# blackle/Megalania

Hardware: AMD Instinct MI355X
Metric: SA neighbour-cost evals/s (higher is better)
Workload: dtype u64

## Files before the change

megalania_amd/csrc/mgl_api.hip:

```cpp
#include "mgl_kernels.hip"
#include "mgl_kernels2.hip"
#include "mgl_kernels3.hip"
#include "mgl_kernels4.hip"
#include "mgl_kernels5.hip"
#include "mgl_pbuild.hip"
#include "mgl_index.hip"
#include "mgl_matchfinder.hip"
#include "mgl_optimal.hip"
#include "mgl_adaptive.hip"
#include "mgl_props.hip"
#include "../../include/megalania_hip.h"

#include <math.h>
#include <stdio.h>
#include <stdlib.h>
#include <string.h>
#include <string>
#include <vector>

static const uint16_t k_cost_table[2048] = {
#include "mgl_cost_table.inc"
};

#define MGL_MAX_INPUT 176000000ull
// ... 412 lines not shown
			hipStream_t st = (h & 1u) ? sa->stream2 : sa->stream;
			hipLaunchKernelGGL((k_neighbours2<false, MGL_NBR_PICK>), dim3((j1 - j0 + sa->pick_waves - 1) / sa->pick_waves), dim3(64 * sa->pick_waves),
			                   (MGL_PICK_T_GLOBAL ? 0u : 4096u) + sa->pick_waves * sa->per_wave_pick, st, sa->ctx,
			                   sa->b2, sa->base.ctl, sa->cfg.seed, step_override, K, sa->nbr, sa->per_wave_pick, sa->d_todo, sa->d_counts,
			                   (unsigned long long*)nullptr, sa->big, sa->d_pickrec, j0, j1, sa->d_pickstate); NBR_TRACE("k_neighbours2<false, MGL_NBR_PICK>");
			hipLaunchKernelGGL((k_neighbours2<false, MGL_NBR_REST>), dim3(j1 - j0), dim3(64), sa->per_wave_rest, st, sa->ctx,
			                   sa->b2, sa->base.ctl, sa->cfg.seed, step_override, K, sa->nbr, sa->per_wave_rest, sa->d_todo, sa->d_counts,
			                   g_prof_big ? (unsigned long long*)nullptr : sa->d_prof, sa->big, sa->d_pickrec, j0, j1, sa->d_pickstate); NBR_TRACE("k_neighbours2<false, MGL_NBR_REST>");
			HIPCHK(hipEventRecord(sa->ev_rest[h], st));
		}
		HIPCHK(hipGetLastError());
		for (uint32_t h = 0; h < slices; h++) {
			const uint32_t j0 = (uint32_t)((uint64_t)K * h / slices), j1 = (uint32_t)((uint64_t)K * (h + 1) / slices);
			HIPCHK(hipStreamWaitEvent(sa->stream3, sa->ev_rest[h], 0));
			if (sa->time_sim_step >= 0 && h < 2) HIPCHK(hipEventRecord(sim_event(sa, 4 * (size_t)sa->time_sim_step + 2 * h), sa->stream3));
			if (sa->count_traffic)
				hipLaunchKernelGGL(k_sim<true>, dim3(j1 - j0), dim3(64 * sa->sim_waves), sim_lds_regular, sa->stream3, sa->ctx, sa->b2, sa->base.ctl,
				                   sa->nbr, sa->big, j0, j1, sa->d_todo3, sa->d_counts + 4, sa->d_traffic);
			else
				hipLaunchKernelGGL(k_sim<false>, dim3(j1 - j0), dim3(64 * sa->sim_waves), sim_lds_regular, sa->stream3, sa->ctx, sa->b2, sa->base.ctl,
				                   sa->nbr, sa->big, j0, j1, sa->d_todo3, sa->d_counts + 4, (unsigned long long*)nullptr);
			NBR_TRACE("k_sim");
			if (sa->time_sim_step >= 0 && h < 2) HIPCHK(hipEventRecord(sim_event(sa, 4 * (size_t)sa->time_sim_step + 2 * h + 1), sa->stream3));
		}
		HIPCHK(hipEventRecord(sa->ev_sim, sa->stream3));
		for (uint32_t h = 1; h < slices; h += 2) HIPCHK(hipStreamWaitEvent(sa->stream, sa->ev_rest[h], 0));
	}
	if (!sa->split_nbr || sa->form_single) {
		hipLaunchKernelGGL((k_neighbours2<false, MGL_NBR_FULL>), dim3(blocks2), dim3(64 * sa->waves_per_block2), sa->nbr2_lds, sa->stream, sa->ctx,
		                   sa->b2, sa->base.ctl, sa->cfg.seed, step_override, K, sa->nbr, sa->per_wave2, sa->d_todo, sa->d_counts,
		                   sa->d_prof, sa->big, sa->d_pickrec, 0u, K, sa->d_pickstate); NBR_TRACE("k_neighbours2<false, MGL_NBR_FULL>");
	}
	const uint32_t bigblocks = sa->big.slots < 1024u ? sa->big.slots : 1024u;
	const uint32_t big_lds = 4096u + sa->per_wave2 + 12u * MGL_BIG_CAP + MGL_COOP_BYTES;
	hipLaunchKernelGGL((k_neighbours2<true, MGL_NBR_FULL>), dim3(bigblocks), dim3(64 * sa->big_waves), big_lds, sa->stream, sa->ctx,
	                   sa->b2, sa->base.ctl, sa->cfg.seed, step_override, K, sa->nbr, sa->per_wave2, sa->d_todo2, sa->d_counts + 1,
	                   g_prof_big ? sa->d_prof : (unsigned long long*)nullptr, sa->big, split_now ? sa->d_pickrec : (uint4*)nullptr, 0u, K, sa->d_pickstate); NBR_TRACE("k_neighbours2<true, MGL_NBR_FULL>");
	if (split_now) {
		HIPCHK(hipStreamWaitEvent(sa->stream, sa->ev_sim, 0));
		BigScratch late = sa->big;
		late.todo_in = sa->d_todo3; late.todo_in_count = sa->d_counts + 4;
		late.cont = nullptr;
		hipLaunchKernelGGL((k_neighbours2<true, MGL_NBR_FULL>), dim3(bigblocks < 64u ? bigblocks : 64u), dim3(64 * sa->big_waves), big_lds, sa->stream, sa->ctx,
		                   sa->b2, sa->base.ctl, sa->cfg.seed, step_override, K, sa->nbr, sa->per_wave2, sa->d_todo2, sa->d_counts + 1,
		                   (unsigned long long*)nullptr, late, sa->d_pickrec, 0u, K, sa->d_pickstate); NBR_TRACE("k_neighbours2<true, MGL_NBR_FULL>");
	}
	const uint32_t blocks = (K + sa->waves_per_block - 1) / sa->waves_per_block;
	hipLaunchKernelGGL(k_neighbours, dim3(blocks < 256u ? blocks : 256u), dim3(64 * sa->waves_per_block), sa->nbr_lds, sa->stream, sa->ctx, sa->base.v,
	                   (const Control*)sa->base.ctl, sa->cfg.seed, step_override, K, sa->nbr, sa->per_wave_bytes,
	                   (const uint32_t*)sa->d_todo2, (const uint32_t*)(sa->d_counts + 1)); NBR_TRACE("k_neighbours");
	HIPCHK(hipGetLastError());
	return MGL_OK;
}

static int import_slab(mgl_sa* sa, const mgl_packet* packets, mgl_pk* d_slab)
{
	HIPCHK(hipMemcpyAsync(sa->d_aos, packets, sizeof(mgl_packet) * (size_t)sa->n, hipMemcpyHostToDevice, sa->stream));
	hipLaunchKernelGGL(k_import, dim3(1024), dim3(256), 0, sa->stream, (const uint32_t*)sa->d_aos, d_slab, sa->n);
	HIPCHK(hipGetLastError());
	return MGL_OK;
}
static int export_slab(mgl_sa* sa, const mgl_pk* d_slab, mgl_packet* packets)
{
	hipLaunchKernelGGL(k_export, dim3(1024), dim3(256), 0, sa->stream, d_slab, sa->d_aos, sa->n);
	HIPCHK(hipGetLastError());
	HIPCHK(hipMemcpyAsync(packets, sa->d_aos, sizeof(mgl_packet) * (size_t)sa->n, hipMemcpyDeviceToHost, sa->stream));
	HIPCHK(hipStreamSynchronize(sa->stream));
// ... 363 lines not shown
			sa->per_wave_rest = (fixed + lists + 15u) & ~15u;
		}
		{
			BigScratch& g = sa->big;
			memset(&g, 0, sizeof g);
			g.chg_cap = sa->chg_cap;
			g.cap = MGL_BIG_CAP; g.uctx_cap = ckpt_elems; g.slots = (uint32_t)(K > 512 ? K : 512);
			HIPCHK(hipMalloc(&g.ins_key, sizeof(uint16_t) * (size_t)g.cap * g.slots));
			HIPCHK(hipMalloc(&g.rem_key, sizeof(uint16_t) * (size_t)g.cap * g.slots));
			HIPCHK(hipMalloc(&g.ins_pos, sizeof(uint32_t) * (size_t)g.cap * g.slots));
			HIPCHK(hipMalloc(&g.rem_pos, sizeof(uint32_t) * (size_t)g.cap * g.slots));
			HIPCHK(hipMalloc(&g.uctx, sizeof(uint16_t) * (size_t)g.uctx_cap * g.slots));
			HIPCHK(hipMalloc(&sa->d_todo2, sizeof(uint32_t) * (K + 1)));
			HIPCHK(hipMemset(sa->d_todo2, 0, sizeof(uint32_t) * (K + 1)));
		}
		{
			uint32_t best_w = 1, best_total = 0;
			for (uint32_t w = 1; w <= 8; w++) {
				const uint32_t bytes = 4096u + w * sa->per_wave2;
				if (bytes > 160u * 1024u) break;
				const uint32_t tot = (160u * 1024u / bytes) * w;
				if (tot > best_total) { best_total = tot; best_w = w; }
			}
			(void)best_w;
			sa->waves_per_block2 = 1;
		}
		sa->nbr2_lds = 4096u + sa->waves_per_block2 * sa->per_wave2;
		sa->build_lds = 4096u + ckpt_elems * 2u + ckpt_elems * 8u;
		HIPCHK(hipMalloc(&sa->d_counts, sizeof(uint32_t) * 16));
		HIPCHK(hipMemset(sa->d_counts, 0, sizeof(uint32_t) * 16));
		HIPCHK(hipMalloc(&sa->d_todo3, sizeof(uint32_t) * (K + 1)));
		HIPCHK(hipMemset(sa->d_todo3, 0, sizeof(uint32_t) * (K + 1)));
		sa->big.todo_in = sa->d_todo; sa->big.todo_in_count = sa->d_counts; sa->big.spill_ctr = sa->d_counts + 2;
		HIPCHK(hipFuncSetAttribute((const void*)k_neighbours2<false, MGL_NBR_FULL>, hipFuncAttributeMaxDynamicSharedMemorySize, (int)sa->nbr2_lds));
		HIPCHK(hipFuncSetAttribute((const void*)k_neighbours2<false, MGL_NBR_PICK>, hipFuncAttributeMaxDynamicSharedMemorySize, 160 * 1024));
		HIPCHK(hipFuncSetAttribute((const void*)k_neighbours2<false, MGL_NBR_REST>, hipFuncAttributeMaxDynamicSharedMemorySize, (int)sa->nbr2_lds));
		HIPCHK(hipFuncSetAttribute((const void*)k_neighbours2<true, MGL_NBR_FULL>, hipFuncAttributeMaxDynamicSharedMemorySize, (int)(4096u + sa->per_wave2 + 12u * MGL_BIG_CAP + MGL_COOP_BYTES)));
		HIPCHK(hipMalloc(&sa->d_pickrec, sizeof(uint4) * K));
		HIPCHK(hipMalloc(&sa->d_pickstate, sizeof(uint4) * 2 * K));
		sa->split_nbr = getenv("MGL_NO_SPLIT") == nullptr;
		if (sa->split_nbr) {
			BigScratch& g = sa->big;
			HIPCHK(hipMalloc(&g.sim_hdr, sizeof(uint4) * (size_t)K));
			HIPCHK(hipMalloc(&g.sim_keys, sizeof(uint16_t) * 2u * sa->chg_cap * (size_t)K));
			HIPCHK(hipMalloc(&g.sim_pos, sizeof(uint32_t) * 2u * sa->chg_cap * (size_t)K));
			HIPCHK(hipMemset(g.sim_hdr, 0xFF, sizeof(uint4) * (size_t)K));
			if (getenv("MGL_NO_CONT") == nullptr) {
				HIPCHK(hipMalloc(&g.cont, sizeof(uint32_t) * MGL_CONT_WORDS * (size_t)g.slots));
				HIPCHK(hipMemset(g.cont, 0, sizeof(uint32_t) * MGL_CONT_WORDS * (size_t)g.slots));
			}
		}
		if (getenv("MGL_SIMW")) { const int w = atoi(getenv("MGL_SIMW")); if (w == 1 || w == 2 || w == 4 || w == 8) sa->sim_waves = (uint32_t)w; }
		sa->adaptive = sa->split_nbr && getenv("MGL_NO_ADAPT") == nullptr;
		sa->form_single = !sa->split_nbr;
		sa->pick_waves = getenv("MGL_PICK_WAVES") ? (uint32_t)atoi(getenv("MGL_PICK_WAVES")) : 0u;
		if (sa->pick_waves != 1 && sa->pick_waves != 2 && sa->pick_waves != 4 && sa->pick_waves != 8) sa->pick_waves = 0;
		{
			uint32_t best_w = 1, best_resident = 0;
			for (uint32_t w = 1; w <= 8; w *= 2) {
				const uint32_t bytes = (MGL_PICK_T_GLOBAL ? 0u : 4096u) + w * sa->per_wave_pick;
				if (bytes > 160u * 1024u) break;
				const uint32_t resident = (160u * 1024u / ((bytes + 1279u) / 1280u * 1280u)) * w;
				if (resident > best_resident) { best_resident = resident; best_w = w; }
			}
			if (n > (1u << 20)) best_w = 1;
			if (sa->pick_waves == 0 || (MGL_PICK_T_GLOBAL ? 0u : 4096u) + sa->pick_waves * sa->per_wave_pick > 160u * 1024u) sa->pick_waves = best_w;
		}
		HIPCHK(hipFuncSetAttribute((const void*)k_sim<false>, hipFuncAttributeMaxDynamicSharedMemorySize, 96 * 1024));
		HIPCHK(hipFuncSetAttribute((const void*)k_sim<true>, hipFuncAttributeMaxDynamicSharedMemorySize, 96 * 1024));
		HIPCHK(hipMalloc(&sa->d_traffic, sizeof(unsigned long long) * 2));
// ... 1261 lines not shown
{
	if (!sa || !out || !bytes) return fail(MGL_EINVAL, "null argument");
	if (!sa->incremental && what != 21 && what != 22) return fail(MGL_EINVAL, "mgl_debug_dump: handle runs the full-walk engine");
	HIPCHK(hipSetDevice(sa->device));
	HIPCHK(hipStreamSynchronize(sa->stream));
	const Base2& b = sa->b2;
	const void* src = nullptr;
	size_t sz = 0;
	uint32_t top = 0;
	if (sa->incremental) HIPCHK(hipMemcpy(&top, b.pool_top, sizeof top, hipMemcpyDeviceToHost));
	switch (what) {
	case 0: src = b.ch_off; sz = sizeof(uint32_t) * sa->ctx.L.total; break;
	case 1: src = b.ch_len; sz = sizeof(uint32_t) * sa->ctx.L.total; break;
	case 2: src = b.ch_pos; sz = sizeof(uint32_t) * (size_t)top; break;
	case 3: src = b.ch_ev; sz = sizeof(uint16_t) * (size_t)top; break;
	case 4: src = b.onwalk; sz = sizeof(uint64_t) * b.nw0; break;
	case 5: src = b.sp0; sz = sizeof(uint64_t) * b.nw0; break;
	case 6: src = b.sp_state; sz = sizeof(uint32_t) * 8 * (size_t)sa->n; break;
	case 7: src = b.ck_probs; sz = sizeof(uint16_t) * (size_t)b.nck * b.ck_elems; break;
	case 8: src = b.ch_cap; sz = sizeof(uint32_t) * sa->ctx.L.total; break;
	case 9: src = sa->d_prof; sz = sa->d_prof ? sizeof(unsigned long long) * (32 + sa->cfg.neighbours_per_step) : 0; break;
	case 80: {
		const uint64_t v[3] = { sa->batch_accepts, sa->batch_fallbacks, sa->batch_early_giveups };
		*bytes = sizeof v;
		if (cap_bytes >= sizeof v) memcpy(out, v, sizeof v);
		return MGL_OK;
	}
	case 84: src = sa->lim.why; sz = sizeof(uint32_t); break;
	case 85: src = b.pool_top; sz = sizeof(uint32_t); break;
	case 83: src = b.ch_sb; sz = sizeof(uint32_t) * (size_t)b.ck_elems * b.sb_stride; break;
	case 81: src = sa->batch.hdr; sz = sizeof(uint32_t) * 16; break;
	case 82: src = sa->batch.acc; sz = sizeof(long long) * 4; break;
	case 10: src = sa->d_counts + 8; sz = sizeof(uint32_t) * 4; break;
	case 14: src = sa->ab.hdr; sz = sa->ab.hdr ? sizeof(uint32_t) * 16 : 0; break;
	case 16: src = sa->base.ctl; sz = sizeof(Control); break;
	case 15: src = sa->d_pickrec; sz = sa->d_pickrec ? sizeof(uint4) * sa->cfg.neighbours_per_step : 0; break;
	case 18: src = sa->d_quad_pos; sz = sizeof(uint32_t) * (sa->n - 1); break;
	case 19: src = sa->d_quad_nx; sz = sizeof(uint16_t) * (sa->n - 1); break;
	case 12: src = sa->d_bucket_off; sz = sizeof(uint32_t) * 65537; break;
	case 13: src = sa->d_bucket_pos; sz = sizeof(uint32_t) * (sa->n - 1); break;
	case 30: case 31: case 32: case 33: case 34: case 35: src = sa->d_xpos[what - 30]; sz = sizeof(uint32_t) * (sa->n - 1); break;
	case 40: case 41: case 42: case 43: case 44: case 45: src = sa->d_xrank[what - 40]; sz = src ? sizeof(uint32_t) * (sa->n - 1) : 0; break;
	case 50: case 51: case 52: case 53: case 54: case 55: src = sa->d_xrun[what - 50]; sz = src ? sizeof(uint32_t) * (sa->n - 1) : 0; break;
	case 60: case 61: case 62: case 63: case 64: case 65: src = sa->d_xnxb[what - 60]; sz = sa->n - 1; break;
	case 70: src = sa->d_oct_pos; sz = sizeof(uint32_t) * (sa->n - 1); break;
	case 71: src = sa->d_oct_rank; sz = sizeof(uint32_t) * (sa->n - 1); break;
	case 72: src = sa->d_oct_run; sz = sizeof(uint32_t) * (sa->n - 1); break;
	case 73: src = sa->d_oct_nx8; sz = sizeof(uint64_t) * (sa->n - 1); break;
	case 74: src = sa->d_hex_pos; sz = sizeof(uint32_t) * (sa->n - 1); break;
	case 75: src = sa->d_hex_rank; sz = sizeof(uint32_t) * (sa->n - 1); break;
	case 76: src = sa->d_hex_run; sz = sizeof(uint32_t) * (sa->n - 1); break;
	case 77: src = sa->d_hex_nx8; sz = sizeof(uint64_t) * (sa->n - 1); break;
	case 22: src = sa->nbr.win2; sz = sizeof(uint32_t) * sa->cfg.neighbours_per_step; break;
	case 21: src = sa->nbr.win; sz = sizeof(uint32_t) * 2 * sa->cfg.neighbours_per_step; break;
	case 11: src = sa->pb.acc; sz = sa->pb.acc ? sizeof(unsigned long long) * 8 : 0; break;
	default: return fail(MGL_EINVAL, "mgl_debug_dump: unknown selector");
	}
	*bytes = sz;
	if (sz > cap_bytes) return fail(MGL_ERANGE, "mgl_debug_dump: buffer too small");
	HIPCHK(hipMemcpy(out, src, sz, hipMemcpyDeviceToHost));
	if (what == 84) HIPCHK(hipMemset(sa->lim.why, 0, sizeof(uint32_t)));
	return MGL_OK;
}

extern "C" int mgl_debug_set(mgl_sa* sa, uint32_t key, uint64_t value)
{
// ... 7 lines not shown
		const uint32_t id = (uint32_t)(value & 0xFFu);
		const uint64_t v = value >> 8;
		if (!sa->incremental || !sa->lim.why) return fail(MGL_EINVAL, "mgl_debug_set: no in-place accept on this handle");
		HIPCHK(hipSetDevice(sa->device));
		HIPCHK(hipStreamSynchronize(sa->stream));
		if (id == 0) {
			if (v) return fail(MGL_EINVAL, "mgl_debug_set: limit id 0 takes value 0 (restore the defaults)");
			for (uint32_t i = 1; i < MGL_LIM_COUNT; i++) sa->lim.v[i] = i == MGL_LIM_SOFT_REACH ? 0u : sa->lim_max.v[i];
		} else {
			if (id >= MGL_LIM_COUNT || v > sa->lim_max.v[id]) return fail(MGL_EINVAL, "mgl_debug_set: unknown limit, or a value above the compiled / allocated one");
			sa->lim.v[id] = (uint32_t)v;
		}
		HIPCHK(hipMemset(sa->lim.why, 0, sizeof(uint32_t)));
		return MGL_OK;
	}
	if (sa && key == 4) {
		if (!sa->d_traffic) return fail(MGL_EINVAL, "mgl_debug_set: no split neighbour evaluation on this handle");
		sa->count_traffic = value != 0;
		return MGL_OK;
	}
	if (!sa) return fail(MGL_EINVAL, "null handle");
	if (key == 0) { sa->ctx.diag_stop = (uint32_t)value; return MGL_OK; }
	if (key == 1) { sa->pb.force_fix = (uint32_t)value; return MGL_OK; }
	if (key == 2) {
		if (value < 8 || value > sa->chg_cap || (value & 7u)) return fail(MGL_EINVAL, "mgl_debug_set: list capacity must be a multiple of 8 within the allocated one");
		sa->big.chg_cap = (uint32_t)value;
		return MGL_OK;
	}
	if (key == 7) {
		if (value != 1 && value != 2 && value != MGL_BIG_WAVES) return fail(MGL_EINVAL, "mgl_debug_set: 1, 2 or MGL_BIG_WAVES wavefronts");
		sa->big_waves = (uint32_t)value;
		return MGL_OK;
	}
	if (key == 3) { sa->force_rollbacks = (uint32_t)value; return MGL_OK; }
	return fail(MGL_EINVAL, "mgl_debug_set: unknown key");
}

#include "mgl_exchange.inc"
```

megalania_amd/csrc/mgl_kernels2.hip:

```cpp
#include "mgl_base2.h"


struct BitAcc {
	uint32_t word;
	uint64_t bits;
};
__device__ __forceinline__ void bitacc_move(BitAcc& a, uint64_t* arr, uint32_t new_word, uint32_t lane)
{
	if (new_word == a.word) return;
	if (lane == 0) arr[a.word] = a.bits;
	for (uint32_t z = a.word + 1 + lane; z < new_word; z += 64) arr[z] = 0;
	a.word = new_word; a.bits = 0;
}

__device__ void build_body(const DevCtx& c, const Base2& b, Control* ctl, int check_cost)
{
	extern __shared__ __attribute__((aligned(16))) unsigned char smem[];
	uint16_t* T = (uint16_t*)smem;
	uint16_t* probs = (uint16_t*)(smem + 4096);
	uint32_t* cnt = (uint32_t*)(smem + 4096 + (size_t)b.ck_elems * 2);
	uint32_t* off = cnt + b.ck_elems;
	const uint32_t lane = threadIdx.x;
	const uint32_t total = c.L.total;
	if (check_cost && !ctl->accepted_flag) return;
// ... 206 lines not shown
		mgl_plan_event(&pl, lane, &ctx, &bit);
		if (INS) { ch.ins_key[n + lane] = (uint16_t)(ctx | (bit << 15)); ch.ins_pos[n + lane] = pos; }
		else { ch.rem_key[n + lane] = (uint16_t)ctx; ch.rem_pos[n + lane] = pos; }
	}
	n += pl.nev;
	const int64_t d = (int64_t)((uint64_t)pl.ndirect << 11);
	ch.direct += INS ? d : -d;
}

__device__ __forceinline__ uint32_t next_with_ctx(const uint16_t* keys, uint32_t start, uint32_t n, uint32_t cx, uint32_t mask)
{
	uint32_t base = start & ~7u;
	while (base < n) {
		const uint4 q = *reinterpret_cast<const uint4*>(keys + base);
		uint4 r = make_uint4(0xFFFFFFFFu, 0xFFFFFFFFu, 0xFFFFFFFFu, 0xFFFFFFFFu);
		if (base + 8u < n) r = *reinterpret_cast<const uint4*>(keys + base + 8u);
		const uint32_t w[8] = { q.x, q.y, q.z, q.w, r.x, r.y, r.z, r.w };
		uint32_t hit = 0;
#pragma unroll
		for (uint32_t e = 0; e < 16; e++) {
			const uint32_t key = (w[e >> 1] >> ((e & 1u) * 16u)) & mask;
			hit |= (key == cx ? 1u : 0u) << e;
		}
		if (base < start) hit &= ~0u << (start - base);
		if (hit) {
			const uint32_t idx = base + (uint32_t)__ffs((int)hit) - 1u;
			return idx < n ? idx : n;
		}
		base += 16;
	}
	return n;
}

__device__ __forceinline__ uint32_t chain_list(Changes& ch, uint32_t lane, bool* too_many)
{
	const uint32_t m = ch.n_ins + ch.n_rem;
	wave_sync();
	for (uint32_t i = lane; i < ch.nbitwords; i += 64) ch.ctxbits[i] = 0;
	wave_sync();
	for (uint32_t e = lane; e < m; e += 64) {
		const uint32_t key = e < ch.n_ins ? (ch.ins_key[e] & 0x7FFFu) : ch.rem_key[e - ch.n_ins];
		atomicOr(&ch.ctxbits[key >> 5], 1u << (key & 31u));
	}
	wave_sync();
	uint32_t nu = 0;
	for (uint32_t wbase = 0; wbase < ch.nbitwords; wbase += 64) {
		const uint32_t word = wbase + lane < ch.nbitwords ? ch.ctxbits[wbase + lane] : 0u;
		const uint32_t cntl = (uint32_t)__popc(word);
		uint32_t incl = cntl;
		for (int o = 1; o < 64; o <<= 1) {
			const uint32_t tmp = (uint32_t)__shfl_up((int)incl, o, 64);
			if ((int)lane >= o) incl += tmp;
		}
		const uint32_t chunk = (uint32_t)__shfl((int)incl, 63, 64);
		if (nu + chunk > ch.uctx_cap) { *too_many = true; return 0; }
		uint32_t at = nu + incl - cntl;
		uint32_t wv = word;
		while (wv) {
			ch.uctx[at++] = (uint16_t)(((wbase + lane) << 5) + ((uint32_t)__ffs((int)wv) - 1u));
			wv &= wv - 1u;
		}
		nu += chunk;
	}
	wave_sync();
	return nu;
}
__device__ __forceinline__ int64_t chain_sim_contexts(const Base2& b, Changes& ch, const uint16_t* T, uint32_t limit, uint16_t* overlay,
                                                      uint32_t lane, uint32_t first, uint32_t stride, uint32_t nu, uint32_t* traffic = nullptr)
{
	int64_t delta = 0;
	for (uint32_t base = first; base < nu; base += stride) {
		if (base + lane >= nu) continue;
		const uint32_t cx = ch.uctx[base + lane];
		uint32_t ii = next_with_ctx(ch.ins_key, 0, ch.n_ins, cx, 0x7FFFu);
		uint32_t ri = next_with_ctx(ch.rem_key, 0, ch.n_rem, cx, 0xFFFFu);
		const uint32_t ipos0 = ii < ch.n_ins ? ch.ins_pos[ii] : MGL_POS_INF;
		const uint32_t rpos0 = ri < ch.n_rem ? ch.rem_pos[ri] : MGL_POS_INF;
		const uint32_t x0 = ipos0 < rpos0 ? ipos0 : rpos0;
		const uint32_t* cpos = b.ch_pos + b.ch_off[cx];
		const uint16_t* cev = b.ch_ev + b.ch_off[cx];
		const uint32_t clen = b.ch_len[cx];
		uint32_t probes = 0;
		uint32_t blo, bhi;
		chain_block(b, cx, x0, &blo, &bhi);
		uint32_t k = chain_lower_bound(cpos, bhi, x0, traffic ? &probes : nullptr, blo);
		if (traffic) *traffic += 20u;
		uint4 c_pa = make_uint4(0, 0, 0, 0), c_pb = c_pa, c_ev = c_pa;
		uint32_t c_base = 0xFFFFFFFFu;
		auto chunk = [&](uint32_t kk) {
			if ((kk & ~7u) != c_base) {
				c_base = kk & ~7u;
				c_pa = *reinterpret_cast<const uint4*>(cpos + c_base);
				c_pb = *reinterpret_cast<const uint4*>(cpos + c_base + 4);
				c_ev = *reinterpret_cast<const uint4*>(cev + c_base);
				if (traffic) *traffic += 48u;
			}
		};
		auto pos_at = [&](uint32_t kk) -> uint32_t {
			const uint32_t e = kk & 7u;
			return e == 0 ? c_pa.x : e == 1 ? c_pa.y : e == 2 ? c_pa.z : e == 3 ? c_pa.w : e == 4 ? c_pb.x : e == 5 ? c_pb.y : e == 6 ? c_pb.z : c_pb.w;
		};
		auto ev_at = [&](uint32_t kk) -> uint32_t {
			const uint32_t e = kk & 7u;
			const uint32_t wd = e < 2 ? c_ev.x : e < 4 ? c_ev.y : e < 6 ? c_ev.z : c_ev.w;
			return (wd >> ((e & 1u) * 16u)) & 0xFFFFu;
		};
		chunk(k);
		uint32_t p = ev_at(k) & 0x7FFu;
		bool at_limit = false, ended = false;
		if (ch.diag == 42) { delta += p; continue; }
		uint32_t iters = 0;
		uint32_t ipos = ipos0, rpos = rpos0;
		for (;;) {
			const bool pending = ipos != MGL_POS_INF || rpos != MGL_POS_INF;
			if (!pending && limit == MGL_POS_INF) break;
			iters++;
			chunk(k);
			const uint32_t bpos = pos_at(k);
			if (ipos < bpos) {
				if (ipos >= limit) { at_limit = true; ended = true; break; }
				const uint32_t bit = ch.ins_key[ii] >> 15;
				delta += T[bit ? 2048u - p : p];
				p = mgl_prob_update(p, bit);
				ii = next_with_ctx(ch.ins_key, ii + 1, ch.n_ins, cx, 0x7FFFu);
				ipos = ii < ch.n_ins ? ch.ins_pos[ii] : MGL_POS_INF;
				continue;
			}
			if (bpos == MGL_POS_INF) { ended = true; break; }
			if (bpos >= limit) { at_limit = true; ended = true; break; }
			const uint32_t ev = ev_at(k);
			const uint32_t bp = ev & 0x7FFu, bb = ev >> 15;
			if (p == bp) {
				if (!pending) { ended = true; break; }
				const uint32_t nxt = ipos < rpos ? ipos : rpos;
				if (nxt > bpos) {
					if (nxt >= limit) { ended = true; break; }
					chain_block(b, cx, nxt, &blo, &bhi);
					k = chain_lower_bound(cpos, bhi, nxt, traffic ? &probes : nullptr, blo > k ? blo : k);
					if (traffic) *traffic += 8u;
					chunk(k);
					p = ev_at(k) & 0x7FFu;
					continue;
				}
			}
			delta -= T[bb ? 2048u - bp : bp];
			if (rpos == bpos) {
				ri = next_with_ctx(ch.rem_key, ri + 1, ch.n_rem, cx, 0xFFFFu);
				rpos = ri < ch.n_rem ? ch.rem_pos[ri] : MGL_POS_INF;
			} else {
				delta += T[bb ? 2048u - p : p];
				p = mgl_prob_update(p, bb);
			}
			k++;
		}
		if (ch.diag == 43) { delta += p; continue; }
		if (!ended) {
			uint32_t kb = k & ~15u;
			uint4 a0 = *reinterpret_cast<const uint4*>(cev + kb);
			uint4 a1 = *reinterpret_cast<const uint4*>(cev + kb + 8);
			int32_t d32 = 0;
			while (!ended) {
				const uint4 n0 = *reinterpret_cast<const uint4*>(cev + kb + 16);
				const uint4 n1 = *reinterpret_cast<const uint4*>(cev + kb + 24);
				if (traffic) *traffic += 32u;
#pragma unroll
				for (uint32_t e = 0; e < 16; e++) {
					const uint32_t idx = kb + e;
					if (ended || idx < k) continue;
					if (idx >= clen) { ended = true; continue; }
					const uint4 q = e < 8 ? a0 : a1;
					const uint32_t h = e & 7u;
					const uint32_t wd = h < 2 ? q.x : h < 4 ? q.y : h < 6 ? q.z : q.w;
					const uint32_t ev = (wd >> ((h & 1u) * 16u)) & 0xFFFFu;
					const uint32_t bp = ev & 0x7FFu, bb = ev >> 15;
					if (p == bp) { ended = true; continue; }
					d32 += (int32_t)T[bb ? 2048u - p : p] - (int32_t)T[bb ? 2048u - bp : bp];
					p = mgl_prob_update(p, bb);
				}
				delta += d32; d32 = 0;
				a0 = n0; a1 = n1; kb += 16;
// ... 147 lines not shown
					mgl_wstate sv = w.st;
					sv.pos = p; sv.ctx_state = lit_steps(w.st.ctx_state, i);
					mgl_plan pl;
					mgl_plan_packet(&c.L, &sv, MGL_LITERAL, 0, 1, byte, 0, prev_byte, &pl);
					if (!__ballot(active && pl.nev != 9u)) {
						uint32_t ctx = 0, bit = 0;
						if (active) mgl_plan_event(&pl, slot, &ctx, &bit);
						for (uint32_t r = 0; r < take; r++) {
							if (active && i == r) probs[ctx] = (uint16_t)mgl_prob_update(probs[ctx], bit);
							wave_sync();
						}
						w.st.pos += take; w.st.ctx_state = lit_steps(w.st.ctx_state, take);
						w.packets += take;
						continue;
					}
				}
			}
			const mgl_pk pk = walk_slab_at(w, w.st.pos);
			walk_packet<true>(w, c, probs, T, mgl_pk_type(pk), mgl_pk_dist(pk), mgl_pk_len(pk), lane);
		}
		wave_sync();
	}
}

__device__ __forceinline__ void walk_from_state(Walk& w, const mgl_wstate& st)
{
	walk_reset(w);
	w.st = st;
}

struct BigScratch {
	uint16_t* ins_key; uint32_t* ins_pos; uint16_t* rem_key; uint32_t* rem_pos; uint16_t* uctx;
	uint32_t cap, uctx_cap, slots;
	const uint32_t* todo_in; const uint32_t* todo_in_count;
	uint32_t* spill_ctr;
	uint32_t chg_cap;
	uint4* sim_hdr;
	uint16_t* sim_keys;
	uint32_t* sim_pos;
	uint32_t* cont;
};
#define MGL_CONT_WORDS 368u
#define MGL_CONT_MAGIC 0x434F4E54u
#ifndef MGL_PICK_T_GLOBAL
#define MGL_PICK_T_GLOBAL 1
#endif
#ifndef MGL_REST_WAVES_PER_SIMD
#define MGL_REST_WAVES_PER_SIMD 4
#endif
#define MGL_NBR_FULL 0
#define MGL_NBR_PICK 1
#define MGL_NBR_REST 2
#ifndef MGL_BIG_WAVES
#define MGL_BIG_WAVES 4u
#endif
#define MGL_COOP_SIM 1u
#define MGL_COOP_EXIT 2u
#define MGL_COOP_BYTES 128u
struct CoopCmd {
	uint32_t gen;
	uint32_t op;
	uint32_t slot;
	uint32_t n_ins, n_rem, nu, limit;
	uint32_t overlay;
	unsigned long long sum[MGL_BIG_WAVES];
};
static_assert(sizeof(CoopCmd) <= MGL_COOP_BYTES, "CoopCmd outgrew its LDS");
__device__ __forceinline__ CoopCmd* coop_cmd(unsigned char* smem, uint32_t per_wave_bytes)
{
	return (CoopCmd*)(smem + 4096u + per_wave_bytes + 12u * MGL_BIG_CAP);
}
__device__ __forceinline__ void coop_share(const DevCtx& c, const Base2& b, const BigScratch& big, unsigned long long* dbg, unsigned char* smem,
                                           uint32_t per_wave_bytes, const uint16_t* T, CoopCmd* cmd, uint32_t lane, uint32_t wid)
{
	const uint32_t slot = uni(cmd->slot), overlay = uni(cmd->overlay);
	Changes cl;
	cl.n_ins = uni(cmd->n_ins); cl.n_rem = uni(cmd->n_rem);
	uint32_t* cp = (uint32_t*)(smem + 4096u + per_wave_bytes);
	cl.ins_pos = cp; cl.rem_pos = cp + MGL_BIG_CAP;
	cl.ins_key = (uint16_t*)(cp + 2u * MGL_BIG_CAP); cl.rem_key = cl.ins_key + MGL_BIG_CAP;
	cl.uctx = big.uctx + (size_t)slot * big.uctx_cap; cl.ctxbits = nullptr;
	cl.cap = MGL_BIG_CAP; cl.uctx_cap = big.uctx_cap; cl.nbitwords = 0;
	cl.direct = 0; cl.dbg = dbg; cl.diag = c.diag_stop; cl.overflow = false; cl.list_full = false;
	const uint16_t* gik = big.ins_key + (size_t)slot * big.cap; const uint32_t* gip = big.ins_pos + (size_t)slot * big.cap;
	const uint16_t* grk = big.rem_key + (size_t)slot * big.cap; const uint32_t* grp = big.rem_pos + (size_t)slot * big.cap;
	for (uint32_t e = threadIdx.x; e < cl.n_ins; e += blockDim.x) { cl.ins_pos[e] = gip[e]; cl.ins_key[e] = gik[e]; }
	for (uint32_t e = threadIdx.x; e < cl.n_rem; e += blockDim.x) { cl.rem_pos[e] = grp[e]; cl.rem_key[e] = grk[e]; }
	__syncthreads();
	const int64_t mine = chain_sim_contexts(b, cl, T, uni(cmd->limit), overlay ? (uint16_t*)(smem + overlay) : nullptr, lane, wid * 64u, blockDim.x, uni(cmd->nu));
	const uint64_t u = wave_sum64((uint64_t)mine);
	if (lane == 0) cmd->sum[wid] = u;
	__syncthreads();
}
__device__ __forceinline__ int64_t coop_sim(const DevCtx& c, const Base2& b, const BigScratch& big, unsigned long long* dbg, unsigned char* smem,
                                            uint32_t per_wave_bytes, const uint16_t* T, Changes& ch, uint32_t slot, uint32_t limit, uint16_t* overlay,
                                            uint32_t lane, bool* too_many)
{
	const uint32_t nu = chain_list(ch, lane, too_many);
	if (*too_many) return 0;
	if (ch.diag == 41) return (int64_t)nu;
	CoopCmd* cmd = coop_cmd(smem, per_wave_bytes);
	if (lane == 0) {
		cmd->op = MGL_COOP_SIM; cmd->slot = slot; cmd->n_ins = ch.n_ins; cmd->n_rem = ch.n_rem; cmd->nu = nu; cmd->limit = limit;
		cmd->overlay = overlay ? (uint32_t)((unsigned char*)overlay - smem) : 0u;
		cmd->gen = cmd->gen + 1u;
	}
	__syncthreads();
	coop_share(c, b, big, dbg, smem, per_wave_bytes, T, cmd, lane, 0u);
	uint64_t d = 0;
	for (uint32_t w = 0; w < (blockDim.x >> 6); w++) d += cmd->sum[w];
	wave_sync();
	return (int64_t)d;
}
__device__ __forceinline__ void coop_helpers(const DevCtx& c, const Base2& b, const BigScratch& big, unsigned long long* dbg, unsigned char* smem,
                                             uint32_t per_wave_bytes, const uint16_t* T, uint32_t lane, uint32_t wid)
{
	CoopCmd* cmd = coop_cmd(smem, per_wave_bytes);
	uint32_t seen = 0;
	for (;;) {
		__syncthreads();
		const uint32_t gen = uni(cmd->gen);
		if (uni(cmd->op) == MGL_COOP_EXIT || gen == seen) return;
		seen = gen;
		coop_share(c, b, big, dbg, smem, per_wave_bytes, T, cmd, lane, wid);
	}
}
template <bool BIG, int MODE>
__device__ __forceinline__ void nbr2_one(const DevCtx& c, const Base2& b, Control* ctl, uint64_t seed,
                                         uint64_t step_override, uint32_t K, const NbrOut& out, uint32_t per_wave_bytes,
                                         uint32_t* todo, uint32_t* todo_count, unsigned long long* prof_acc,
                                         const BigScratch& big, uint4* pickrec, uint32_t j_base, uint32_t j_end, uint4* pickstate,
                                         unsigned char* smem, const uint16_t* T, uint32_t unit, uint32_t lane, uint32_t wid)
{
	uint32_t j = j_base + unit;
	uint32_t slot = 0;
	const unsigned long long t_begin = prof_acc ? __builtin_readcyclecounter() : 0ull;
	if (BIG) {
		slot = unit;
		const uint32_t nflag = *big.todo_in_count;
		if (slot >= nflag) return;
		j = uni(big.todo_in[slot]);
		if (lane == 0) atomicAdd((unsigned long long*)&ctl->big_nbrs, 1ull);
	}
	if (j >= K || (!BIG && j >= j_end)) return;
	unsigned char* mine = smem + ((MODE == MGL_NBR_REST || (MODE == MGL_NBR_PICK && MGL_PICK_T_GLOBAL)) ? 0u : 4096u) + (size_t)wid * per_wave_bytes;
	Journal jn;
	jn.old = (mgl_pk*)mine;
	jn.neu = jn.old + MGL_MAX_DIFFS;
	jn.pos = (uint32_t*)(jn.neu + MGL_MAX_DIFFS);
	jn.count = 0; jn.overflow = false;
	Changes ch;
	ch.nbitwords = (c.L.total + 31u) >> 5;
	ch.ctxbits = jn.pos + MGL_MAX_DIFFS;
	unsigned char* uni_base = MODE == MGL_NBR_PICK ? mine : (unsigned char*)(ch.ctxbits + ((ch.nbitwords + 3u) & ~3u));
	uint16_t* probs = (uint16_t*)uni_base;
	uint32_t* lencost = (uint32_t*)(uni_base + (size_t)b.ck_elems * 2);
	ch.ins_pos = (uint32_t*)uni_base;
// ... 586 lines not shown
```

Measured before the change: 14.50 million.

## Index big-neighbour change lists by context and build unique-context list cooperatively

For large change lists in the cooperative big-neighbour simulation, the workgroup builds a per-list index of (context, position) entries in LDS and bitonic-sorts it. Each lane then binary-searches for its context's group and steps through it, instead of linearly scanning the whole list with next_with_ctx. The unique-context list is now built by all waves through an LDS bitmap, atomicOr and a wave prefix scan, replacing the single-wave chain_list. This adds LDS per block and sort and sync overhead, and it adds debug atomic counters on every indexed call.

After: 14.43 million. Within noise of the previous version (-0.5%).

```diff
diff --git a/megalania_amd/csrc/mgl_api.hip b/megalania_amd/csrc/mgl_api.hip
--- a/megalania_amd/csrc/mgl_api.hip
+++ b/megalania_amd/csrc/mgl_api.hip
@@ -468,7 +468,7 @@
 		                   sa->d_prof, sa->big, sa->d_pickrec, 0u, K, sa->d_pickstate); NBR_TRACE("k_neighbours2<false, MGL_NBR_FULL>");
 	}
 	const uint32_t bigblocks = sa->big.slots < 1024u ? sa->big.slots : 1024u;
-	const uint32_t big_lds = 4096u + sa->per_wave2 + 12u * MGL_BIG_CAP + MGL_COOP_BYTES;
+	const uint32_t big_lds = MGL_BIG_LDS(sa->per_wave2);
 	hipLaunchKernelGGL((k_neighbours2<true, MGL_NBR_FULL>), dim3(bigblocks), dim3(64 * sa->big_waves), big_lds, sa->stream, sa->ctx,
 	                   sa->b2, sa->base.ctl, sa->cfg.seed, step_override, K, sa->nbr, sa->per_wave2, sa->d_todo2, sa->d_counts + 1,
 	                   g_prof_big ? sa->d_prof : (unsigned long long*)nullptr, sa->big, split_now ? sa->d_pickrec : (uint4*)nullptr, 0u, K, sa->d_pickstate); NBR_TRACE("k_neighbours2<true, MGL_NBR_FULL>");
@@ -898,10 +898,12 @@
 		HIPCHK(hipMalloc(&sa->d_todo3, sizeof(uint32_t) * (K + 1)));
 		HIPCHK(hipMemset(sa->d_todo3, 0, sizeof(uint32_t) * (K + 1)));
 		sa->big.todo_in = sa->d_todo; sa->big.todo_in_count = sa->d_counts; sa->big.spill_ctr = sa->d_counts + 2;
+		sa->big.index_min = MGL_INDEX_MIN;
+		if (MGL_BIG_LDS(sa->per_wave2) > 160u * 1024u) return fail(MGL_EINVAL, "second pass: its workgroup's LDS exceeds a CU's 160 KiB");
 		HIPCHK(hipFuncSetAttribute((const void*)k_neighbours2<false, MGL_NBR_FULL>, hipFuncAttributeMaxDynamicSharedMemorySize, (int)sa->nbr2_lds));
 		HIPCHK(hipFuncSetAttribute((const void*)k_neighbours2<false, MGL_NBR_PICK>, hipFuncAttributeMaxDynamicSharedMemorySize, 160 * 1024));
 		HIPCHK(hipFuncSetAttribute((const void*)k_neighbours2<false, MGL_NBR_REST>, hipFuncAttributeMaxDynamicSharedMemorySize, (int)sa->nbr2_lds));
-		HIPCHK(hipFuncSetAttribute((const void*)k_neighbours2<true, MGL_NBR_FULL>, hipFuncAttributeMaxDynamicSharedMemorySize, (int)(4096u + sa->per_wave2 + 12u * MGL_BIG_CAP + MGL_COOP_BYTES)));
+		HIPCHK(hipFuncSetAttribute((const void*)k_neighbours2<true, MGL_NBR_FULL>, hipFuncAttributeMaxDynamicSharedMemorySize, (int)MGL_BIG_LDS(sa->per_wave2)));
 		HIPCHK(hipMalloc(&sa->d_pickrec, sizeof(uint4) * K));
 		HIPCHK(hipMalloc(&sa->d_pickstate, sizeof(uint4) * 2 * K));
 		sa->split_nbr = getenv("MGL_NO_SPLIT") == nullptr;
@@ -2229,6 +2231,7 @@
 	case 81: src = sa->batch.hdr; sz = sizeof(uint32_t) * 16; break;
 	case 82: src = sa->batch.acc; sz = sizeof(long long) * 4; break;
 	case 10: src = sa->d_counts + 8; sz = sizeof(uint32_t) * 4; break;
+	case 17: src = sa->d_counts + 13; sz = sizeof(uint32_t) * 3; break;
 	case 14: src = sa->ab.hdr; sz = sa->ab.hdr ? sizeof(uint32_t) * 16 : 0; break;
 	case 16: src = sa->base.ctl; sz = sizeof(Control); break;
 	case 15: src = sa->d_pickrec; sz = sa->d_pickrec ? sizeof(uint4) * sa->cfg.neighbours_per_step : 0; break;
@@ -2302,6 +2305,11 @@
 		sa->big_waves = (uint32_t)value;
 		return MGL_OK;
 	}
+	if (key == 8) {
+		if (value > 0xFFFFFFFFull) return fail(MGL_EINVAL, "mgl_debug_set: list length out of range");
+		sa->big.index_min = (uint32_t)value;
+		return MGL_OK;
+	}
 	if (key == 3) { sa->force_rollbacks = (uint32_t)value; return MGL_OK; }
 	return fail(MGL_EINVAL, "mgl_debug_set: unknown key");
 }
diff --git a/megalania_amd/csrc/mgl_kernels2.hip b/megalania_amd/csrc/mgl_kernels2.hip
--- a/megalania_amd/csrc/mgl_kernels2.hip
+++ b/megalania_amd/csrc/mgl_kernels2.hip
@@ -262,6 +262,53 @@
 	return n;
 }
 
+static_assert(MGL_BIG_CAP <= 4096u, "a list index takes 12 bits of an index entry");
+struct ListIndex {
+	const uint32_t* ins;
+	const uint32_t* rem;
+};
+__device__ __forceinline__ uint32_t group_start(const uint32_t* idx, uint32_t n, uint32_t cx)
+{
+	const uint32_t want = cx << 12;
+	uint32_t lo = 0, hi = n;
+	while (lo < hi) {
+		const uint32_t mid = (lo + hi) >> 1;
+		if (idx[mid] < want) lo = mid + 1u; else hi = mid;
+	}
+	return lo;
+}
+__device__ __forceinline__ uint32_t group_entry(const uint32_t* idx, uint32_t g, uint32_t n, uint32_t cx)
+{
+	if (g >= n) return n;
+	const uint32_t v = idx[g];
+	return (v >> 12) == cx ? (v & 0xFFFu) : n;
+}
+__device__ __forceinline__ uint32_t pow2_at_least(uint32_t n)
+{
+	return n <= 1u ? 1u : 1u << (32u - (uint32_t)__clz((int)(n - 1u)));
+}
+__device__ __forceinline__ void coop_index_sort(uint32_t* si, uint32_t pi, uint32_t* sr, uint32_t pr)
+{
+	const uint32_t pmax = pi > pr ? pi : pr;
+	for (uint32_t k = 2; k <= pmax; k <<= 1) {
+		for (uint32_t j = k >> 1; j > 0; j >>= 1) {
+			for (uint32_t t = threadIdx.x; t < (pmax >> 1); t += blockDim.x) {
+				const uint32_t a = ((t & ~(j - 1u)) << 1) | (t & (j - 1u)), b = a | j;
+				const bool up = (a & k) == 0;
+				if (k <= pi && b < pi) {
+					const uint32_t x = si[a], y = si[b];
+					if ((x > y) == up) { si[a] = y; si[b] = x; }
+				}
+				if (k <= pr && b < pr) {
+					const uint32_t x = sr[a], y = sr[b];
+					if ((x > y) == up) { sr[a] = y; sr[b] = x; }
+				}
+			}
+			__syncthreads();
+		}
+	}
+}
+
 __device__ __forceinline__ uint32_t chain_list(Changes& ch, uint32_t lane, bool* too_many)
 {
 	const uint32_t m = ch.n_ins + ch.n_rem;
@@ -295,15 +342,25 @@
 	wave_sync();
 	return nu;
 }
+template <bool IDX = false>
 __device__ __forceinline__ int64_t chain_sim_contexts(const Base2& b, Changes& ch, const uint16_t* T, uint32_t limit, uint16_t* overlay,
-                                                      uint32_t lane, uint32_t first, uint32_t stride, uint32_t nu, uint32_t* traffic = nullptr)
+                                                      uint32_t lane, uint32_t first, uint32_t stride, uint32_t nu, uint32_t* traffic = nullptr,
+                                                      ListIndex li = ListIndex{ nullptr, nullptr })
 {
 	int64_t delta = 0;
+	const bool grouped = IDX && li.ins != nullptr;
 	for (uint32_t base = first; base < nu; base += stride) {
 		if (base + lane >= nu) continue;
 		const uint32_t cx = ch.uctx[base + lane];
-		uint32_t ii = next_with_ctx(ch.ins_key, 0, ch.n_ins, cx, 0x7FFFu);
-		uint32_t ri = next_with_ctx(ch.rem_key, 0, ch.n_rem, cx, 0xFFFFu);
+		uint32_t gi = 0, gr = 0;
+		uint32_t ii, ri;
+		if (grouped) {
+			gi = group_start(li.ins, ch.n_ins, cx); ii = group_entry(li.ins, gi, ch.n_ins, cx);
+			gr = group_start(li.rem, ch.n_rem, cx); ri = group_entry(li.rem, gr, ch.n_rem, cx);
+		} else {
+			ii = next_with_ctx(ch.ins_key, 0, ch.n_ins, cx, 0x7FFFu);
+			ri = next_with_ctx(ch.rem_key, 0, ch.n_rem, cx, 0xFFFFu);
+		}
 		const uint32_t ipos0 = ii < ch.n_ins ? ch.ins_pos[ii] : MGL_POS_INF;
 		const uint32_t rpos0 = ri < ch.n_rem ? ch.rem_pos[ri] : MGL_POS_INF;
 		const uint32_t x0 = ipos0 < rpos0 ? ipos0 : rpos0;
@@ -352,7 +409,8 @@
 				const uint32_t bit = ch.ins_key[ii] >> 15;
 				delta += T[bit ? 2048u - p : p];
 				p = mgl_prob_update(p, bit);
-				ii = next_with_ctx(ch.ins_key, ii + 1, ch.n_ins, cx, 0x7FFFu);
+				if (grouped) ii = group_entry(li.ins, ++gi, ch.n_ins, cx);
+				else ii = next_with_ctx(ch.ins_key, ii + 1, ch.n_ins, cx, 0x7FFFu);
 				ipos = ii < ch.n_ins ? ch.ins_pos[ii] : MGL_POS_INF;
 				continue;
 			}
@@ -375,7 +433,8 @@
 			}
 			delta -= T[bb ? 2048u - bp : bp];
 			if (rpos == bpos) {
-				ri = next_with_ctx(ch.rem_key, ri + 1, ch.n_rem, cx, 0xFFFFu);
+				if (grouped) ri = group_entry(li.rem, ++gr, ch.n_rem, cx);
+				else ri = next_with_ctx(ch.rem_key, ri + 1, ch.n_rem, cx, 0xFFFFu);
 				rpos = ri < ch.n_rem ? ch.rem_pos[ri] : MGL_POS_INF;
 			} else {
 				delta += T[bb ? 2048u - p : p];
@@ -589,6 +648,7 @@
 struct BigScratch {
 	uint16_t* ins_key; uint32_t* ins_pos; uint16_t* rem_key; uint32_t* rem_pos; uint16_t* uctx;
 	uint32_t cap, uctx_cap, slots;
+	uint32_t index_min;
 	const uint32_t* todo_in; const uint32_t* todo_in_count;
 	uint32_t* spill_ctr;
 	uint32_t chg_cap;
@@ -611,15 +671,24 @@
 #ifndef MGL_BIG_WAVES
 #define MGL_BIG_WAVES 4u
 #endif
+#ifndef MGL_COOP_LIST
+#define MGL_COOP_LIST 1
+#endif
 #define MGL_COOP_SIM 1u
 #define MGL_COOP_EXIT 2u
 #define MGL_COOP_BYTES 128u
+#define MGL_INDEX_BYTES (8u * MGL_BIG_CAP)
+#define MGL_BIG_LDS(per_wave) (4096u + (per_wave) + 12u * MGL_BIG_CAP + MGL_COOP_BYTES + MGL_INDEX_BYTES)
+#ifndef MGL_INDEX_MIN
+#define MGL_INDEX_MIN 512u
+#endif
 struct CoopCmd {
 	uint32_t gen;
 	uint32_t op;
 	uint32_t slot;
 	uint32_t n_ins, n_rem, nu, limit;
 	uint32_t overlay;
+	uint32_t bits;
 	unsigned long long sum[MGL_BIG_WAVES];
 };
 static_assert(sizeof(CoopCmd) <= MGL_COOP_BYTES, "CoopCmd outgrew its LDS");
@@ -627,8 +696,8 @@
 {
 	return (CoopCmd*)(smem + 4096u + per_wave_bytes + 12u * MGL_BIG_CAP);
 }
-__device__ __forceinline__ void coop_share(const DevCtx& c, const Base2& b, const BigScratch& big, unsigned long long* dbg, unsigned char* smem,
-                                           uint32_t per_wave_bytes, const uint16_t* T, CoopCmd* cmd, uint32_t lane, uint32_t wid)
+__device__ __forceinline__ uint32_t coop_share(const DevCtx& c, const Base2& b, const BigScratch& big, unsigned long long* dbg, unsigned char* smem,
+                                               uint32_t per_wave_bytes, const uint16_t* T, CoopCmd* cmd, uint32_t lane, uint32_t wid, bool* too_many)
 {
 	const uint32_t slot = uni(cmd->slot), overlay = uni(cmd->overlay);
 	Changes cl;
@@ -636,34 +705,102 @@
 	uint32_t* cp = (uint32_t*)(smem + 4096u + per_wave_bytes);
 	cl.ins_pos = cp; cl.rem_pos = cp + MGL_BIG_CAP;
 	cl.ins_key = (uint16_t*)(cp + 2u * MGL_BIG_CAP); cl.rem_key = cl.ins_key + MGL_BIG_CAP;
-	cl.uctx = big.uctx + (size_t)slot * big.uctx_cap; cl.ctxbits = nullptr;
-	cl.cap = MGL_BIG_CAP; cl.uctx_cap = big.uctx_cap; cl.nbitwords = 0;
+	cl.uctx = big.uctx + (size_t)slot * big.uctx_cap; cl.ctxbits = (uint32_t*)(smem + uni(cmd->bits));
+	cl.cap = MGL_BIG_CAP; cl.uctx_cap = big.uctx_cap; cl.nbitwords = (c.L.total + 31u) >> 5;
 	cl.direct = 0; cl.dbg = dbg; cl.diag = c.diag_stop; cl.overflow = false; cl.list_full = false;
 	const uint16_t* gik = big.ins_key + (size_t)slot * big.cap; const uint32_t* gip = big.ins_pos + (size_t)slot * big.cap;
 	const uint16_t* grk = big.rem_key + (size_t)slot * big.cap; const uint32_t* grp = big.rem_pos + (size_t)slot * big.cap;
-	for (uint32_t e = threadIdx.x; e < cl.n_ins; e += blockDim.x) { cl.ins_pos[e] = gip[e]; cl.ins_key[e] = gik[e]; }
-	for (uint32_t e = threadIdx.x; e < cl.n_rem; e += blockDim.x) { cl.rem_pos[e] = grp[e]; cl.rem_key[e] = grk[e]; }
+	const bool indexed = cl.n_ins + cl.n_rem >= big.index_min;
+	uint32_t* si = (uint32_t*)(smem + 4096u + per_wave_bytes + 12u * MGL_BIG_CAP + MGL_COOP_BYTES);
+	uint32_t* sr = si + MGL_BIG_CAP;
+	const uint32_t pi = pow2_at_least(cl.n_ins), pr = pow2_at_least(cl.n_rem);
+	for (uint32_t e = threadIdx.x; e < cl.n_ins; e += blockDim.x) {
+		const uint16_t key = gik[e];
+		cl.ins_pos[e] = gip[e]; cl.ins_key[e] = key;
+		if (indexed) si[e] = ((uint32_t)(key & 0x7FFFu) << 12) | e;
+	}
+	for (uint32_t e = threadIdx.x; e < cl.n_rem; e += blockDim.x) {
+		const uint16_t key = grk[e];
+		cl.rem_pos[e] = grp[e]; cl.rem_key[e] = key;
+		if (indexed) sr[e] = ((uint32_t)key << 12) | e;
+	}
+	if (indexed) {
+		for (uint32_t e = cl.n_ins + threadIdx.x; e < pi; e += blockDim.x) si[e] = 0xFFFFFFFFu;
+		for (uint32_t e = cl.n_rem + threadIdx.x; e < pr; e += blockDim.x) sr[e] = 0xFFFFFFFFu;
+	}
+	if (MGL_COOP_LIST) for (uint32_t i = threadIdx.x; i < cl.nbitwords; i += blockDim.x) cl.ctxbits[i] = 0;
 	__syncthreads();
-	const int64_t mine = chain_sim_contexts(b, cl, T, uni(cmd->limit), overlay ? (uint16_t*)(smem + overlay) : nullptr, lane, wid * 64u, blockDim.x, uni(cmd->nu));
+	uint32_t nu = uni(cmd->nu);
+	bool many = false;
+	if (MGL_COOP_LIST) {
+		for (uint32_t e = threadIdx.x; e < cl.n_ins; e += blockDim.x) { const uint32_t key = cl.ins_key[e] & 0x7FFFu; atomicOr(&cl.ctxbits[key >> 5], 1u << (key & 31u)); }
+		for (uint32_t e = threadIdx.x; e < cl.n_rem; e += blockDim.x) { const uint32_t key = cl.rem_key[e]; atomicOr(&cl.ctxbits[key >> 5], 1u << (key & 31u)); }
+		__syncthreads();
+		const uint32_t waves = blockDim.x >> 6;
+		nu = 0;
+		for (uint32_t wbase = 0, trip = 0; wbase < cl.nbitwords; wbase += 64, trip++) {
+			const uint32_t word = wbase + lane < cl.nbitwords ? cl.ctxbits[wbase + lane] : 0u;
+			const uint32_t cntl = (uint32_t)__popc(word);
+			uint32_t incl = cntl;
+			for (int o = 1; o < 64; o <<= 1) {
+				const uint32_t tmp = (uint32_t)__shfl_up((int)incl, o, 64);
+				if ((int)lane >= o) incl += tmp;
+			}
+			if (trip % waves == wid) {
+				uint32_t at = nu + incl - cntl;
+				uint32_t wv = word;
+				while (wv) {
+					if (at < cl.uctx_cap) cl.uctx[at] = (uint16_t)(((wbase + lane) << 5) + ((uint32_t)__ffs((int)wv) - 1u));
+					at++;
+					wv &= wv - 1u;
+				}
+			}
+			nu += (uint32_t)__shfl((int)incl, 63, 64);
+		}
+		nu = uni(nu);
+		many = nu > cl.uctx_cap;
+		__syncthreads();
+	}
+	*too_many = many;
+	int64_t mine = 0;
+	if (!many && cl.diag != 41) {
+		if (indexed) {
+			coop_index_sort(si, pi, sr, pr);
+			if (threadIdx.x == 0) {
+				atomicAdd(big.spill_ctr + 3, 1u);
+				if (cl.n_ins == 0 || cl.n_rem == 0) atomicAdd(big.spill_ctr + 4, 1u);
+				if (((cl.n_ins | cl.n_rem) & 15u) != 0) atomicAdd(big.spill_ctr + 5, 1u);
+			}
+		}
+		const ListIndex li = { indexed ? si : nullptr, indexed ? sr : nullptr };
+		mine = chain_sim_contexts<true>(b, cl, T, uni(cmd->limit), overlay ? (uint16_t*)(smem + overlay) : nullptr, lane, wid * 64u, blockDim.x, nu, nullptr, li);
+	}
 	const uint64_t u = wave_sum64((uint64_t)mine);
 	if (lane == 0) cmd->sum[wid] = u;
 	__syncthreads();
+	return nu;
 }
 __device__ __forceinline__ int64_t coop_sim(const DevCtx& c, const Base2& b, const BigScratch& big, unsigned long long* dbg, unsigned char* smem,
                                             uint32_t per_wave_bytes, const uint16_t* T, Changes& ch, uint32_t slot, uint32_t limit, uint16_t* overlay,
                                             uint32_t lane, bool* too_many)
 {
-	const uint32_t nu = chain_list(ch, lane, too_many);
-	if (*too_many) return 0;
-	if (ch.diag == 41) return (int64_t)nu;
+	uint32_t nu = 0;
+	if (!MGL_COOP_LIST) {
+		nu = chain_list(ch, lane, too_many);
+		if (*too_many) return 0;
+		if (ch.diag == 41) return (int64_t)nu;
+	}
 	CoopCmd* cmd = coop_cmd(smem, per_wave_bytes);
 	if (lane == 0) {
 		cmd->op = MGL_COOP_SIM; cmd->slot = slot; cmd->n_ins = ch.n_ins; cmd->n_rem = ch.n_rem; cmd->nu = nu; cmd->limit = limit;
 		cmd->overlay = overlay ? (uint32_t)((unsigned char*)overlay - smem) : 0u;
+		cmd->bits = (uint32_t)((unsigned char*)ch.ctxbits - smem);
 		cmd->gen = cmd->gen + 1u;
 	}
 	__syncthreads();
-	coop_share(c, b, big, dbg, smem, per_wave_bytes, T, cmd, lane, 0u);
+	nu = coop_share(c, b, big, dbg, smem, per_wave_bytes, T, cmd, lane, 0u, too_many);
+	if (*too_many) return 0;
+	if (ch.diag == 41) return (int64_t)nu;
 	uint64_t d = 0;
 	for (uint32_t w = 0; w < (blockDim.x >> 6); w++) d += cmd->sum[w];
 	wave_sync();
@@ -679,7 +816,8 @@
 		const uint32_t gen = uni(cmd->gen);
 		if (uni(cmd->op) == MGL_COOP_EXIT || gen == seen) return;
 		seen = gen;
-		coop_share(c, b, big, dbg, smem, per_wave_bytes, T, cmd, lane, wid);
+		bool too_many;
+		coop_share(c, b, big, dbg, smem, per_wave_bytes, T, cmd, lane, wid, &too_many);
 	}
 }
 template <bool BIG, int MODE>
```
